# sakarias88/racer-tracer

Hardware: AMD Instinct MI355X
Metric: Msamples/s (W*H*spp/s) at 1920x1080 (higher is better)
Workload: dtype f64; 1 GPU; cornell_box.yml 1920x1080 1024spp max_depth 20; strip_rows=8, parallelism=image rows interleaved over 1 GPU(s)

## Files before the change

### racer-tracer_amd/csrc/rt_api.hip

```cpp
#include <hip/hip_runtime.h>
#include <stdint.h>
#include <stdio.h>
#include <string.h>
#include <algorithm>
#include <cmath>
#include <atomic>
#include <string>
#include <vector>
#include <thread>
#include <chrono>
#include "rt_scene.h"

extern "C" hipError_t rtdev_launch_post_rgba8(const RtToneMap *tm, const double *rgb, size_t n_pixels, uint8_t *rgba,
                                              double *mapped, hipStream_t stream);

using rtapi::Cancel;
using rtapi::Delivery;
using rtapi::chunk_plan;
using rtapi::fail;
using rtapi::owned_rows_of;

namespace {

int fill_args(const RtScene *s, const RtCamera *c, const RtRenderParams *p, rtdev::TraceArgs &a) {
// ... 184 lines not shown
    a.slice_rows = a.owned_rows;
    const size_t slice_elems = (size_t)p->width * (size_t)a.slice_rows * 3;
    if (b.partial.count < slice_elems * (size_t)a.total_chunks) RT_HIP(b.partial.alloc(slice_elems * (size_t)a.total_chunks));
    if (b.queue.count < n_launches) RT_HIP(b.queue.alloc(n_launches));
    a.partial = b.partial.ptr;
    RT_HIP(hipMemsetAsync(b.segments.ptr, 0, rtdev::RT_STAT_SLOTS * sizeof(unsigned long long), stream));
#ifdef RT_PROFILE_REGIONS
    RT_HIP(hipMemsetAsync(b.segments.ptr + rtdev::RT_STAT_WALL + 0, 0xff, sizeof(unsigned long long), stream));
    RT_HIP(hipMemsetAsync(b.segments.ptr + rtdev::RT_STAT_WALL + 2, 0xff, sizeof(unsigned long long), stream));
#endif
    RT_HIP(hipMemsetAsync(b.queue.ptr, 0, sizeof(unsigned int) * b.queue.count, stream));
    const int rc = order_bvh_for_camera(s, camera, stream);
    if (rc != RT_OK) return rc;
    RT_HIP(hipEventRecord(b.ev_begin, stream));
    return RT_OK;
}

int launch_pool(RtScene *s, rtdev::TraceArgs &a, const std::vector<int> &starts, int first_chunk, int n_chunks, int index,
                unsigned max_blocks, hipStream_t stream, const uint32_t *tile_list = nullptr, uint32_t n_list = 0) {
    if (tile_list && (a.n_regions > 1 || n_list > (uint32_t)a.n_tiles))
        return fail(RT_ERR_INVALID_ARGUMENT, "a tile list is for one-region launches, at most one entry per tile");
    a.sample_begin = starts[(size_t)first_chunk];
    a.sample_end = starts[(size_t)(first_chunk + n_chunks)];
    a.n_chunks = n_chunks;
    a.chunk_base = first_chunk;
    a.tile_list = tile_list;
    a.n_list = tile_list ? n_list : 0u;
    const uint32_t tiles = tile_list ? n_list : (uint32_t)a.n_tiles;
    a.n_items = (uint32_t)a.n_chunks * tiles;
    if ((uint64_t)a.n_chunks * (uint64_t)tiles >= 0x40000000ull)
        return fail(RT_ERR_UNSUPPORTED, "more than 2^30 work items in one launch");
    a.queue = s->buf.queue.ptr + index;
    const unsigned blocks = std::min(max_blocks, (a.n_items + 3) / 4);
    RT_HIP(s->kernels->trace_pool(&a, s->prims_class, s->textured, s->specular, s->use_bvh, blocks, stream));
    return RT_OK;
}

int enqueue_pool(RtScene *s, rtdev::TraceArgs &a, const RtCamera *camera, const RtRenderParams *p, double *out_device,
                 hipStream_t stream, int batch, const Cancel &cancel, const Delivery *delivery, int out_col_step,
                 int out_cols, int &launches) {
    std::vector<int> starts;
    unsigned max_blocks = 0;
    int rc = setup_pool_grid(s, a, p, starts, max_blocks);
    if (rc != RT_OK) return rc;
    const int total_chunks = a.total_chunks;
    const std::vector<rtapi::Launch> plan = rtapi::plan_launches(starts, batch);
    if (delivery) {
        if (plan.size() != 1 || p->scale > 1) return fail(RT_ERR_UNSUPPORTED, "a delivering launch is one whole-frame launch");
        if ((rc = setup_delivery(s, a, *delivery, total_chunks, stream)) != RT_OK) return rc;
    }
    rtapi::RenderBuffers &b = s->buf;
    if ((rc = pool_prologue(s, a, camera, p, plan.size(), cancel.armed() || (delivery && delivery->cancellable), stream)) != RT_OK)
        return rc;
    int chunks_done = 0;
    for (const rtapi::Launch &l : plan) {
        if (cancel.raised()) return RT_ERR_CANCEL_EVENT;
        if ((rc = launch_pool(s, a, starts, l.first_chunk, l.n_chunks, launches, max_blocks, stream)) != RT_OK) return rc;
        chunks_done += a.n_chunks;
        ++launches;
    }
    RT_HIP(hipEventRecord(b.ev_traced, stream));
    if (!delivery)
        RT_HIP(s->kernels->resolve_chunks(b.partial.ptr, out_device, p->width, p->height, chunks_done, a.slice_rows, a.strip_rows,
                                          a.strip_count, a.strip_index, a.step_x, a.step_y, a.cover_w, a.cover_h, out_col_step,
                                          out_cols, p->samples, stream));
    RT_HIP(hipEventRecord(b.ev_resolved, stream));
    return RT_OK;
// ... 261 lines not shown
```

### racer-tracer_amd/csrc/rt_pool_coop.h

```cpp
#pragma once
#include "rt_pool_lds.h"

namespace RT_KNS {

__device__ __forceinline__ int lane_rank(uint64_t mask) {
    return (int)__builtin_amdgcn_mbcnt_hi((uint32_t)(mask >> 32), __builtin_amdgcn_mbcnt_lo((uint32_t)mask, 0u));
}

__device__ __forceinline__ void post_request(SphereSlot *slot, const ScatterPrefix &P, uint32_t base) {
    __hip_atomic_store(&slot->b, P.b, __ATOMIC_RELAXED, __HIP_MEMORY_SCOPE_WAVEFRONT);
    __hip_atomic_store(&slot->y, P.y, __ATOMIC_RELAXED, __HIP_MEMORY_SCOPE_WAVEFRONT);
    __hip_atomic_store(&slot->x, P.x, __ATOMIC_RELAXED, __HIP_MEMORY_SCOPE_WAVEFRONT);
    __hip_atomic_store(&slot->w, P.w, __ATOMIC_RELAXED, __HIP_MEMORY_SCOPE_WAVEFRONT);
    __hip_atomic_store(&slot->z, P.z, __ATOMIC_RELAXED, __HIP_MEMORY_SCOPE_WAVEFRONT);
    __hip_atomic_store(&slot->base, base, __ATOMIC_RELAXED, __HIP_MEMORY_SCOPE_WAVEFRONT);
}
__device__ __forceinline__ void move_masked(const d3 &p, uint64_t mask, d3 &v) {
    uint64_t saved;
    asm volatile("s_and_saveexec_b64 %[saved], %[mask]\n\t"
                 "v_mov_b64 %[x], %[px]\n\t"
                 "v_mov_b64 %[y], %[py]\n\t"
                 "v_mov_b64 %[z], %[pz]\n\t"
                 "s_mov_b64 exec, %[saved]"
                 : [x] "+v"(v.x), [y] "+v"(v.y), [z] "+v"(v.z), [saved] "=&s"(saved)
                 : [mask] "s"(mask), [px] "v"(p.x), [py] "v"(p.y), [pz] "v"(p.z)
                 : "scc");
}
__device__ __forceinline__ void increment_masked(uint32_t &v, uint64_t mask) {
    asm("v_addc_co_u32 %[v], vcc, 0, %[v], %[mask]" : [v] "+v"(v) : [mask] "s"(mask) : "vcc");
}
__device__ __forceinline__ uint64_t lowest_in_groups(uint64_t x, int lg) {
    const int q = 1 << lg;
    uint64_t low = 1;
#pragma unroll
    for (int k = 0; k < 6; ++k) low |= low << ((q << k) & 63);
    const uint64_t top = low << (q - 1);
    return x & (((~x & ~top) + low) ^ (~x & top));
}

template <bool PAIRS>
__device__ __forceinline__ void closest_hit_rects(const Prim *table, const d3 &o, const d3 &d, const d3 &inv_d, double &best_t, int &best) {
    auto test_plane = [&](auto axis, const Prim &P, int i) {
#ifndef RT_EXACT_DIV
        rect_closest_update<decltype(axis)::value>(P.p[0], P.p[1], P.p[2], P.p[3], P.p[4], o, d, inv_d, 0.001, best_t, best, i);
        return;
#endif
        double t;
        if (rect_t<true>(decltype(axis)::value, P.p[0], P.p[1], P.p[2], P.p[3], P.p[4], o, d, inv_d, 0.001, best_t, t)) {
            best_t = t;
            best = i;
        }
    };
    const Prim *rec = table;
    int i = 0;
    auto group = [&](auto axis, int end) {
        if (PAIRS) {
            for (; i + 1 < end; i += 2, rec += 2) {
                const Prim pa = load_prim_uniform(rec, 0), pb = load_prim_uniform(rec, 1);
                test_plane(axis, pa, i);
                test_plane(axis, pb, i + 1);
            }
            if (i < end) {
                test_plane(axis, load_prim_uniform(rec, 0), i);
                ++i;
                ++rec;
            }
        } else {
            for (; i < end; ++i, ++rec) test_plane(axis, load_prim_uniform(rec, 0), i);
        }
    };
    const RT_CONSTANT TraceArgs *KB = kernargs_here();
    const int end_xy = KB->rect_end[0], end_xz = KB->rect_end[1], end_yz = KB->rect_end[2];
    group(std::integral_constant<int, 2>(), end_xy);
    group(std::integral_constant<int, 1>(), end_xz);
    group(std::integral_constant<int, 0>(), end_yz);
}

template <int MAX_ROUNDS>
__device__ __forceinline__ uint64_t coop_random_in_unit_sphere(uint64_t pending, uint32_t pixel, uint32_t sample, uint32_t seg,
                                                           uint32_t &base, uint32_t k0, uint32_t k1, int lane,
                                                           SphereSlot *slot, d3 &result) {
    uint64_t have = 0;
    const ScatterPrefix own = scatter_prefix(pixel, sample, seg, k0, k1);
    for (int round = 0; round < MAX_ROUNDS && pending != 0; ++round) {
        const int n = __popcll(pending);
        if (round > 0 && n < 8) break;
        const int lg = n > 32 ? 0 : (n > 16 ? 1 : (n > 8 ? 2 : (n > 4 ? 3 : (n > 2 ? 4 : (n > 1 ? 5 : 6)))));
        d3 cand;
        uint64_t take;
        if (lg == 0) {
            const d3 p = sphere_candidate(philox_from_prefix(own, base, k0, k1));
            cand = p;
            take = pending;
            const uint64_t inside = ballot(len2(p) < 1.0);
            have |= pending & inside;
            pending &= ~inside;
            if (__builtin_amdgcn_inverse_ballot_w64(pending)) base += 1u;
        } else {
            const bool need = __builtin_amdgcn_inverse_ballot_w64(pending);
            const int rank = lane_rank(pending);
            if (need) post_request(slot + rank, own, base);
// ... 127 lines not shown
```

### racer-tracer_amd/csrc/rt_pool_lds.h

```cpp
#pragma once
#include "rt_trace_common.h"

namespace RT_KNS {

struct NoiseSlots {
    double p[8][3];
    int depth[8];
    int perlin[8];
    double term[8][8];
};
struct alignas(16) Req4 {
    uint32_t x, y, z, w;
};
struct alignas(8) SphereSlot {
    uint32_t b, y, x, w, z, base;
};
static_assert(sizeof(SphereSlot) == 3 * sizeof(double), "a slot holds the request or the sample");

template <bool TEXTURED> union SamplerScratch {
    Req4 req[32];
    SphereSlot sphere[32];
    NoiseSlots noise;
};
template <> union SamplerScratch<false> {
    Req4 req[32];
    SphereSlot sphere[32];
};

struct alignas(16) ItemInfo {
    int chunk, tx, ty, tile_py0, region, reg_tiles, rows_aligned, _pad;
};

template <bool TEXTURED, int NBUF, bool OVERLAP> struct WaveLds {
    double base[OVERLAP ? 1 : 64][3];
    double u[OVERLAP ? 64 : 1];
    double sum[OVERLAP ? 128 : 64][3];
    SamplerScratch<TEXTURED> scratch;
    uint8_t pix_of[64];
    double v[NBUF][64];
    ItemInfo info[2];
    double ulc[3];
};

enum : uint32_t { RING_SLOTS = 92u };
struct PretraceLds {
    double cam_origin[3], bg_top[3];
    double u[64];
    double sum[64][3];
    SamplerScratch<false> scratch;
    uint8_t pix_of[64];
    double ring_v[RING_SLOTS];
    double ring_t[RING_SLOTS];
    uint32_t ring_w[RING_SLOTS];
    uint16_t ring_best[RING_SLOTS];
    uint32_t n_started;
    ItemInfo info[1];
    double ulc[3];
};

}
```

### racer-tracer_amd/csrc/rt_primary_bounds.h

```cpp
#pragma once
#include <cmath>
#include <stdint.h>

namespace rtdev {

struct PixelRect {
    int32_t px0, px1, py0, py1;
};

inline PixelRect primary_bounds(const double origin[3], const double ulc[3], const double horizontal[3], const double vertical[3],
                                double lens_radius, int width, int height, const double mn[3], const double mx[3]) {
    const PixelRect whole = {0, width - 1, 0, height - 1};
    const double kPad = 1.0;
    if (width < 2 || height < 2) return whole;
    if (!(lens_radius == 0.0)) return whole;
    for (int k = 0; k < 3; ++k) {
        if (!std::isfinite(origin[k]) || !std::isfinite(ulc[k]) || !std::isfinite(horizontal[k]) || !std::isfinite(vertical[k]))
            return whole;
        if (!std::isfinite(mn[k]) || !std::isfinite(mx[k]) || mn[k] > mx[k]) return whole;
    }
    const double a[3] = {horizontal[0], horizontal[1], horizontal[2]};
    const double b[3] = {-vertical[0], -vertical[1], -vertical[2]};
    const double r[3] = {origin[0] - ulc[0], origin[1] - ulc[1], origin[2] - ulc[2]};
    auto det3 = [](const double p[3], const double q[3], const double s[3]) {
        return p[0] * (q[1] * s[2] - q[2] * s[1]) - p[1] * (q[0] * s[2] - q[2] * s[0]) + p[2] * (q[0] * s[1] - q[1] * s[0]);
    };
    auto norm3 = [](const double p[3]) { return std::sqrt(p[0] * p[0] + p[1] * p[1] + p[2] * p[2]); };
    double u_min = INFINITY, u_max = -INFINITY, v_min = INFINITY, v_max = -INFINITY;
    for (int corner = 0; corner < 8; ++corner) {
        double c[3];
        for (int k = 0; k < 3; ++k) c[k] = -(((corner >> k) & 1 ? mx[k] : mn[k]) - origin[k]);
        const double det = det3(a, b, c);
        if (!std::isfinite(det) || !(std::fabs(det) > 1e-9 * norm3(a) * norm3(b) * norm3(c))) return whole;
        const double u = det3(r, b, c) / det, v = det3(a, r, c) / det, lambda = det3(a, b, r) / det;
        if (!std::isfinite(u) || !std::isfinite(v) || !std::isfinite(lambda) || !(lambda > 0.0)) return whole;
        u_min = std::fmin(u_min, u);
        u_max = std::fmax(u_max, u);
        v_min = std::fmin(v_min, v);
        v_max = std::fmax(v_max, v);
    }
    auto low = [&](double t, int n) { return (int32_t)std::fmin(std::fmax(std::floor(t * (double)(n - 1)) - 1.0 - kPad, 0.0), (double)n); };
    auto high = [&](double t, int n) { return (int32_t)std::fmax(std::fmin(std::ceil(t * (double)(n - 1)) + kPad, (double)(n - 1)), -1.0); };
    return PixelRect{low(u_min, width), high(u_max, width), low(v_min, height), high(v_max, height)};
}

}
```

### racer-tracer_amd/csrc/rt_scene.h

```cpp
#pragma once
#include <hip/hip_runtime.h>
#include <stdint.h>
#include <string>
#include <vector>
#include "rt_device_types.h"
#include "rt_bvh.h"
#include "rt_error.h"
#include "rt_plan.h"
#include "../../include/rt_abi.h"

#define RT_LAUNCHER_LIST(X)                                                                                                \
    X(trace, rtdev_launch_trace, hipError_t,                                                                               \
      (const rtdev::TraceArgs *args, int prims_class, int textured, int specular, hipStream_t stream))                     \
    X(resolve, rtdev_launch_resolve, hipError_t,                                                                           \
      (const double *accum, double *out, int width, int height, int strip_rows, int strip_count, int strip_index,         \
       int samples, hipStream_t stream))                                                                                   \
    X(pool_blocks_per_cu, rtdev_pool_blocks_per_cu, int,                                                                   \
      (int prims_class, int textured, int specular, int bvh, size_t dyn_lds))                                              \
    X(pool_static_lds, rtdev_pool_static_lds, int, (int prims_class, int textured, int specular, int bvh))                 \
    X(trace_pool, rtdev_launch_trace_pool, hipError_t,                                                                     \
      (const rtdev::TraceArgs *args, int prims_class, int textured, int specular, int bvh, unsigned blocks,               \
       hipStream_t stream))                                                                                                \
    X(resolve_chunks, rtdev_launch_resolve_chunks, hipError_t,                                                             \
      (const double *partial, double *out, int width, int height, int n_chunks, int slice_rows, int strip_rows,           \
       int strip_count, int strip_index, int step_x, int step_y, int cover_w, int cover_h, int out_col_step, int out_cols, \
       int samples, hipStream_t stream))                                                                                   \
    X(fold_chunks, rtdev_launch_fold_chunks, hipError_t,                                                                   \
      (const double *partial, double *running, double *out, size_t n, int c0, int c1, int samples_done,                   \
       hipStream_t stream))                                                                                                \
    X(fold_adaptive, rtdev_launch_fold_adaptive, hipError_t, (const rtdev::AdaptiveFold *f, hipStream_t stream))           \
    X(nee, rtdev_launch_nee, hipError_t,                                                                                   \
      (const rtdev::TraceArgs *args, const rtdev::NeeArgs *nee, int prims_class, int textured, int specular, int bvh,     \
       hipStream_t stream))                                                                                                \
    X(nee_pass, rtdev_launch_nee_pass, hipError_t,                                                                         \
      (const rtdev::TraceArgs *args, const rtdev::NeeArgs *nee, int prims_class, int textured, int specular, int bvh,     \
       hipStream_t stream))                                                                                                \
    X(nee_chunk, rtdev_launch_nee_chunk, hipError_t,                                                                       \
      (const double *running, double *boundary, double *squares, size_t n, int samples, hipStream_t stream))              \
    X(nee_decide, rtdev_launch_nee_decide, hipError_t, (const rtdev::NeeDecide *f, hipStream_t stream))                    \
    X(nee_stream, rtdev_launch_nee_stream, hipError_t,                                                                     \
      (const rtdev::TraceArgs *args, const rtdev::NeeArgs *nee, int prims_class, int textured, int specular, int bvh,     \
       unsigned blocks, hipStream_t stream))                                                                               \
    X(nee_stream_blocks_per_cu, rtdev_nee_stream_blocks_per_cu, int,                                                       \
      (int prims_class, int textured, int specular, int bvh))                                                              \
    X(nee_stream_chunk, rtdev_nee_stream_chunk, int, (void))
#define RT_DECLARE_LAUNCHER(member, name, ret, params) \
    extern "C" ret name params;                        \
    extern "C" ret name##_exact params;
RT_LAUNCHER_LIST(RT_DECLARE_LAUNCHER)
#undef RT_DECLARE_LAUNCHER

namespace rtapi {

struct Launchers {
#define RT_LAUNCHER_MEMBER(member, name, ret, params) ret(*member) params;
// ... 101 lines not shown
        for (hipEvent_t *evs : {ev_pass_begin, ev_pass_traced, ev_folded, ev_counted, ev_copied})
            for (int k = 0; k < 3; ++k)
                if (evs[k]) (void)hipEventDestroy(evs[k]);
        if (stream_copy) (void)hipStreamDestroy(stream_copy);
        *this = RenderBuffers();
    }
};

}

extern "C" hipError_t rtdev_launch_guides(const rtdev::TraceArgs *args, const RtGuides *guides, hipStream_t stream);
extern "C" hipError_t rtdev_launch_denoise_step(const RtDenoiseParams *d, int step, int width, int height, const double *in,
                                                const RtGuides *guides, double *out, hipStream_t stream);

struct RtScene {
    int device = 0;
    rtapi::DevBuf<rtdev::Prim> prims;
    rtapi::DevBuf<rtdev::Texture> textures;
    rtapi::DevBuf<rtdev::Image> images;
    rtapi::DevBuf<rtdev::Perlin> perlins;
    std::vector<uint8_t *> image_pixels;
    int n_prims = 0, n_materials = 0, n_textures = 0, n_images = 0, n_perlins = 0;
    int perlin_identity = 1;
    rtdev::Background bg;
    int prims_class = 2;
    int rect_end[3] = {0, 0, 0};
    int sphere_end = 0;
    int box_end = 0;
    int textured = 0;
    double radiance_bound = 0.0;
    int specular = 0;
    int has_moving = 0;
    double box_mn[3] = {1.0, 1.0, 1.0}, box_mx[3] = {-1.0, -1.0, -1.0};

    int use_bvh = 0;
    rtapi::DevBuf<rtdev::BvhNode> bvh_nodes;
    rtapi::DevBuf<rtdev::BvhNode> bvh_nodes_ordered;
    rtapi::DevBuf<int32_t> bvh_prim_index;
    rtapi::DevBuf<rtdev::LeafGeo> leaf_geo;
    double leaf_time_a = 0.0, leaf_inv_dt = 1.0;
    int n_bvh_nodes = 0;
    double bvh_root_mn[3] = {0, 0, 0}, bvh_root_mx[3] = {0, 0, 0}, bvh_center[3] = {0, 0, 0};
    bool bvh_nodes_in_lds = false;
    rtdev::BvhBuild bvh_host;
    double bvh_ordered_for[3] = {0, 0, 0};
    bool bvh_is_ordered = false;
    std::vector<rtdev::BvhNode> bvh_ordered_nodes[2];
    int bvh_upload_slot = 0;

    bool use_v1 = false;
    bool exact = false;
    const rtapi::Launchers *kernels = nullptr;
    bool gather_staged = false;
    int num_cus = 0, pool_blocks_per_cu = 1;
    int pool_blocks_per_cu_lens = 1;
    int pool_static_lds = 0;
    size_t pool_dyn_lds = 0, pool_dyn_lds_lens = 0;

    std::vector<int32_t> lights;
    rtapi::DevBuf<int32_t> nee_slot, nee_prim;

    rtapi::RenderBuffers buf;
    bool has_stats = false;
    int last_launches = 0;
    bool summed_times = false;
    double summed_kernel_ms = 0.0, summed_resolve_ms = 0.0;
// ... 75 lines not shown
```

### racer-tracer_amd/csrc/rt_scene_create.hip

```cpp
#include <hip/hip_runtime.h>
#include <stdint.h>
#include <string.h>
#include <memory>
#include <mutex>
#include <string>
#include <vector>
#include "rt_scene.h"

using rtapi::DevBuf;
using rtapi::fail;

namespace {
struct CachedSet {
    int device;
    rtapi::RenderBuffers buf;
};
std::mutex g_cache_mutex;
std::vector<CachedSet> g_cache;
const size_t kCachedSetsPerDevice = 2;

void render_cache_put(RtScene *s) {
    if (s->buf.complete()) {
        std::lock_guard<std::mutex> lock(g_cache_mutex);
        size_t held = 0;
// ... 159 lines not shown

    std::vector<rtdev::Prim> prims = rtapi::pack_prims(d);
    s->radiance_bound = rtapi::scene_radiance_bound(d);
    const std::vector<rtdev::Perlin> perlins = rtapi::pack_perlins(d, s->perlin_identity);
    const rtapi::Selection sel = rtapi::select_variant(d);
    s->prims_class = sel.prims_class;
    s->textured = sel.textured;
    s->specular = sel.specular;
    s->has_moving = sel.has_moving;
    rtapi::scene_bounds(d, s->box_mn, s->box_mx);
    s->use_bvh = d->n_primitives > rtapi::kBvhThreshold;
    if (opt.closest_hit != RT_HIT_AUTO) s->use_bvh = opt.closest_hit == RT_HIT_BVH && d->n_primitives > 0;
    if (s->radiance_bound == 0.0 && !s->use_v1 && (s->use_bvh || s->prims_class == 2)) s->exact = true;
    s->kernels = s->exact ? &kExactLaunchers : &kFastLaunchers;
    if (!s->use_bvh && (size_t)d->n_primitives * sizeof(rtdev::Prim) > rtapi::kLinearTableBytes)
        return fail(RT_ERR_UNSUPPORTED, "RT_HIT_LINEAR: the primitive table does not fit in LDS");

    std::vector<int32_t> order((size_t)d->n_primitives);
    for (size_t j = 0; j < order.size(); ++j) order[j] = (int32_t)j;
    rtdev::BvhBuild bvh;
    rtapi::LeafTable leaves;
    if (s->use_bvh) {
        bvh = choose_bvh(d, s);
        order.assign(bvh.prim_index.begin(), bvh.prim_index.end());
        std::vector<rtdev::Prim> ordered(prims.size());
        for (size_t j = 0; j < bvh.prim_index.size(); ++j) ordered[j] = prims[(size_t)bvh.prim_index[j]];
        prims.swap(ordered);
        leaves = rtapi::leaf_geometry(prims);
    } else {
        const rtapi::LinearGroups groups = rtapi::group_linear_table(prims, order);
        for (int g = 0; g < 3; ++g) s->rect_end[g] = groups.rect_end[g];
        s->sphere_end = groups.sphere_end;
        s->box_end = groups.box_end;
    }
    const rtapi::LightTables lights = rtapi::light_tables(d, order, rtapi::kMaxLights);

    std::vector<rtdev::Image> images;
    if ((rc = upload_images(d, s, images)) != RT_OK) return rc;
    const std::vector<rtdev::Texture> textures = rtapi::pack_textures(d, images);
    if (s->use_bvh && (rc = upload_bvh(s, bvh, leaves)) != RT_OK) return rc;
    if ((rc = rtapi::build_light_list(s, lights)) != RT_OK) return rc;
    if ((rc = upload(s->prims, prims)) != RT_OK) return rc;
    if ((rc = upload(s->textures, textures)) != RT_OK) return rc;
    if ((rc = upload(s->images, images)) != RT_OK) return rc;
    if ((rc = upload(s->perlins, perlins)) != RT_OK) return rc;
    s->n_prims = d->n_primitives;
    s->n_materials = d->n_materials;
    s->n_textures = d->n_textures;
    s->n_images = d->n_images;
    s->n_perlins = d->n_perlins;
    s->bg.kind = d->background.kind;
    for (int k = 0; k < 3; ++k) {
        s->bg.top[k] = d->background.top[k];
        s->bg.bottom[k] = d->background.bottom[k];
    }
    if ((rc = size_pool(s)) != RT_OK) return rc;
    if ((rc = acquire_render_buffers(s)) != RT_OK) return rc;
    *out = half_built.release();
    return RT_OK;
}

}

extern "C" {

void rt_scene_destroy(RtScene *s) {
// ... 78 lines not shown
```

### racer-tracer_amd/csrc/rt_trace_pool_kernel.hip

```cpp
#include <cstddef>
#include <type_traits>
#include "rt_trace_common.h"
#include "rt_variant_dispatch.h"
#include "rt_pool_profile.h"
#include "rt_pool_lds.h"
#include "rt_pool_coop.h"
#include "rt_pool_deliver.h"

#ifndef RT_OCC_TEX
#define RT_OCC_TEX 4
#endif
#ifndef RT_OCC_TEX_BVH
#define RT_OCC_TEX_BVH 4
#endif
#ifndef RT_OCC_TEX_ANY
#define RT_OCC_TEX_ANY 4
#endif
#ifndef RT_OCC_SPEC
#define RT_OCC_SPEC 5
#endif
#ifndef RT_OCC_ANY
#define RT_OCC_ANY 5
#endif
#ifndef RT_OCC_PLAIN
#define RT_OCC_PLAIN 7
#endif
namespace RT_KNS {

template <int PRIMS, bool TEXTURED, bool SPECULAR, bool BVH>
__global__ __launch_bounds__(256, TEXTURED ? (PRIMS == PRIMS_ANY ? (BVH ? RT_OCC_TEX_BVH : RT_OCC_TEX_ANY) : RT_OCC_TEX) : (BVH ? 4 : (PRIMS == PRIMS_ANY ? RT_OCC_ANY : (SPECULAR ? RT_OCC_SPEC : RT_OCC_PLAIN)))) void k_trace_pool_f64(const TraceArgs A) {
    constexpr int NBUF = BVH ? 1 : 2;
#if defined(RT_EXACT_DIV) || defined(RT_NO_OVERLAP)
    constexpr bool OVERLAP = false;
#else
    constexpr bool OVERLAP = BVH || PRIMS == PRIMS_ANY;
#endif
#ifdef RT_NO_PRETRACE
    constexpr bool PRETRACE = false;
#else
    constexpr bool PRETRACE = PRIMS == PRIMS_RECTS && !TEXTURED && !SPECULAR && !BVH;
#endif
    using Lds = std::conditional_t<PRETRACE, PretraceLds, WaveLds<TEXTURED, NBUF, OVERLAP>>;
    __shared__ Lds lds_all[4];
    extern __shared__ __align__(16) unsigned char dyn_lds[];
    struct PerlinGradients {
        double ranvec[256][3];
    };
    static_assert(offsetof(Perlin, ranvec) == 0, "the gradients lead the Perlin record");
    const Perlin *lds_perlin = nullptr;
    if (TEXTURED) {
        if (A.perlin_in_lds) {
            const size_t at = BVH ? (size_t)A.bvh_lds_nodes * sizeof(BvhNode)
                                  : (size_t)A.n_prims * sizeof(Prim) + (size_t)A.n_textures * sizeof(Texture);
            const uint64_t *src = reinterpret_cast<const uint64_t *>(A.perlins);
            uint64_t *dst = reinterpret_cast<uint64_t *>(dyn_lds + at);
            for (int i = threadIdx.x; i < (int)(sizeof(PerlinGradients) / 8); i += 256) dst[i] = src[i];
            lds_perlin = reinterpret_cast<const Perlin *>(dyn_lds + at);
        }
        __syncthreads();
    }
    double (*lens)[64][2] = nullptr;
    if (A.lens_lds) {
        size_t at = BVH ? (size_t)A.bvh_lds_nodes * sizeof(BvhNode)
// ... 106 lines not shown
        uint32_t tile = local - chunk * reg_tiles;
        if (tile_list != nullptr) tile = (uint32_t)__builtin_amdgcn_readfirstlane((int)tile_list[tile]);
        const int ty = reg_ty0 + (int)(tile / (uint32_t)reg_ntx);
        const int tx = reg_tx0 + (int)(tile % (uint32_t)reg_ntx);
        const int cur = (int)(state >> 6) & 1;
        int n_smp;
        {
            const RT_CONSTANT TraceArgs *K = kernargs_here();
            smp0 = K->chunk_start[A.chunk_base + (int)chunk];
            n_smp = K->chunk_start[A.chunk_base + (int)chunk + 1] - smp0;
        }

        const bool rows_aligned = A.strip_count <= 1 || (A.strip_rows & 7) == 0;
        tile_py0 = ty * 8 * A.step_y;
        if (A.strip_count > 1 && rows_aligned) {
            const int q = (ty * 8) / A.strip_rows;
            tile_py0 = (q * A.strip_count + A.strip_index) * A.strip_rows + (ty * 8 - q * A.strip_rows);
        }
        const int my_px = (tx * 8 + (lane & 7)) * A.step_x;
        const int my_vrow = ty * 8 + (lane >> 3);
        int my_py = tile_py0 + (lane >> 3) * A.step_y;
        if (!rows_aligned)
            my_py = ((my_vrow / A.strip_rows) * A.strip_count + A.strip_index) * A.strip_rows + my_vrow % A.strip_rows;
        const bool my_valid = my_px < A.cover_w && my_vrow < A.owned_rows && my_py < A.height;
        my_pixel = (uint32_t)my_py * (uint32_t)A.width + (uint32_t)my_px;
        const uint64_t valid_mask = ballot(my_valid);
        n_valid = __popcll(valid_mask);
        bool culled = false;
        if constexpr (PRETRACE) {
            const RT_CONSTANT TraceArgs *K = kernargs_here();
            const int x0 = K->cull_px0, x1 = K->cull_px1, y0 = K->cull_py0, y1 = K->cull_py1;
            const uint64_t seen = valid_mask & ballot(my_px >= x0) & ballot(my_px <= x1) & ballot(my_py >= y0) & ballot(my_py <= y1);
            culled = seen == 0ull && K->bg.kind != RT_BG_SKY && K->max_depth >= 1;
        }
        {
            if (!culled) {
                uint32_t pixel_stream = RT_RNG_SAMPLE_PIXEL;
                if constexpr (PRETRACE) asm volatile("" : "+s"(pixel_stream));
                PathRng prng{my_pixel, pixel_stream, A.seed_lo, A.seed_hi};
                u4 bj = prng.block(0, RT_RNG_PIXEL, 0);
                const RT_CONSTANT TraceArgs *K = kernargs_here();
                const double u = div_by((double)my_px + u53(bj.a, bj.b), (double)(A.width - 1), K->inv_width_m1);
                if constexpr (OVERLAP || PRETRACE) {
                    L.u[lane] = u;
                } else {
                    const d3 base = ld3(K->cam.ulc) + u * ld3(K->cam.horizontal);
                    L.base[lane][0] = base.x;
                    L.base[lane][1] = base.y;
                    L.base[lane][2] = base.z;
                }
            }
            unsigned long long zero = FIXED_SUMS ? 0ull - (unsigned long long)n_smp * 0x4330000000000000ull : 0ull;
            if constexpr (PRETRACE) asm volatile("" : "+v"(zero));
            unsigned long long *sum = reinterpret_cast<unsigned long long *>(L.sum[cur * 64 + lane]);
            sum[0] = zero;
            sum[1] = zero;
            sum[2] = zero;
            if (my_valid) L.pix_of[lane_rank(valid_mask)] = lane;
            if (lane == 0) L.info[cur] = ItemInfo{(int)chunk, tx, ty, tile_py0, region, (int)reg_tiles, rows_aligned ? 1 : 0, 0};
        }
        if constexpr (PRETRACE) {
            if (culled) {
                const d3 bg = ld3(L.bg_top);
                if (bg.x != 0.0 || bg.y != 0.0 || bg.z != 0.0)
                    for (int k = 0; k < n_smp; ++k) {
                        atomicAdd(&L.sum[lane_of_wave][0], bg.x);
// ... 118 lines not shown
                atomicAdd(&L.sum[pix_b][0], one);
                atomicAdd(&L.sum[pix_b][1], one);
                atomicAdd(&L.sum[pix_b][2], one);
            }
            if (lane == 0) L.n_started += (uint32_t)__popcll(in_pool);
            next += (uint32_t)__popcll(in_pool);
            return;
        }
        const u4 bc = philox4x32(pixel_b, sample_b, RT_RNG_CAMERA, 0u, A.seed_lo, A.seed_hi);
        const uint32_t in_ring = min(b << 6, total) - next;
        uint32_t park = ring_head + in_ring + (uint32_t)lane;
        if (park >= RING_SLOTS) park -= RING_SLOTS;
        d3 bo, bd;
        {
            const double v = div_by((double)py_b + u53(bc.a, bc.b), (double)(A.height - 1), K->inv_height_m1);
            double lx, ly;
            asm volatile("" : "=v"(lx), "=v"(ly));
            if (kernargs_here()->lens_lds != 0) {
                lx = ly = 0.0;
                uint32_t w_here = w;
                asm volatile("" : "+v"(w_here));
                coop_random_in_unit_disk(w_here < total, pixel_b, sample_b, A.seed_lo, A.seed_hi, lane, L.scratch.req, lx, ly);
                lx = lx * K->cam.lens_radius;
                ly = ly * K->cam.lens_radius;
                lens_ring[park][0] = lx;
                lens_ring[park][1] = ly;
            }
            L.ring_v[park] = v;
            camera_ray(pix_b, v, lx, ly, bo, bd);
        }
        double best_t = __builtin_inf();
        int best = -1;
        increment_masked(n_segments, in_pool);
        closest_hit_rects<false>(A.prims, bo, bd, rcp3(bd), best_t, best);
        d3 C = ld3(L.bg_top);
        if (kernargs_here()->bg.kind == RT_BG_SKY) {
            const double t = 0.5 * (unit_fast(bd).y + 1.0);
            C = (1.0 - t) * C + t * ld3(kernargs_here()->bg.bottom);
        }
        const uint64_t hit = in_pool & ballot(best >= 0);
        int kind;
        asm volatile("" : "=v"(kind));
        if (__builtin_amdgcn_inverse_ballot_w64(hit)) {
            const Material &M = lds_prims[best].mat;
            kind = M.kind;
            C = ld3(M.color);
        }
        asm volatile("" : "+v"(kind));
        const uint64_t light = hit & ballot(kind == RT_MAT_DIFFUSE_LIGHT);
        const uint64_t ends = kernargs_here()->max_depth <= 1 ? in_pool : (in_pool & ~hit) | light;
        const uint64_t lives = in_pool & ~ends;
        if (__builtin_amdgcn_inverse_ballot_w64(ends)) {
            atomicAdd(&L.sum[pix_b][0], C.x);
            atomicAdd(&L.sum[pix_b][1], C.y);
            atomicAdd(&L.sum[pix_b][2], C.z);
        }
        if (lane == 0) L.n_started += (uint32_t)__popcll(in_pool);
        uint32_t slot = ring_head + in_ring + (uint32_t)lane_rank(lives);
        if (slot >= RING_SLOTS) slot -= RING_SLOTS;
        if (__builtin_amdgcn_inverse_ballot_w64(lives)) {
            const double v = L.ring_v[park];
            double lx, ly;
            asm volatile("" : "=v"(lx), "=v"(ly));
            if (kernargs_here()->lens_lds != 0) {
                lx = lens_ring[park][0];
                ly = lens_ring[park][1];
            }
            asm volatile("" ::: "memory");
            L.ring_v[slot] = v;
            L.ring_t[slot] = best_t;
            L.ring_w[slot] = w;
            L.ring_best[slot] = (uint16_t)best;
            if (kernargs_here()->lens_lds != 0) {
                lens_ring[slot][0] = lx;
                lens_ring[slot][1] = ly;
            }
        }
        next += (uint32_t)__popcll(ends);
        }
    };

    uint64_t alive_m = 0;
    int spix = 0;
    PathRng rng{0, 0, A.seed_lo, A.seed_hi};
    d3 o = mk(0, 0, 0), d = o, T = o;
    uint32_t seg = 0;
    double ray_time = 0.0;
    uint64_t waiting_m = 0;
// ... 526 lines not shown
    if (lane == 0 && total_segments) atomicAdd(A.segments + RT_STAT_SEGMENTS, total_segments);
    if constexpr (PRETRACE) {
        int first = lane_of_wave;
        asm volatile("" : "+v"(first));
        n_started = first == 0 ? L.n_started : 0u;
    }
    unsigned long long started = n_started;
#pragma unroll
    for (int off = 32; off > 0; off >>= 1) started += __shfl_down(started, off, 64);
    if (lane == 0 && started) atomicAdd(A.segments + RT_STAT_SAMPLES, started);
}

}

#if defined(RT_BB_COUNT) && !defined(RT_EXACT_DIV)
enum { RT_BB_MAX = 8192 };
extern "C" {
__device__ __attribute__((used)) unsigned long long rt_bb_counts[RT_BB_MAX];
int rtdev_bb_counts(unsigned long long *out, int n, int reset) {
    if (n > RT_BB_MAX) n = RT_BB_MAX;
    if (hipDeviceSynchronize() != hipSuccess) return -1;
    if (out && hipMemcpyFromSymbol(out, HIP_SYMBOL(rt_bb_counts), (size_t)n * sizeof(unsigned long long)) != hipSuccess) return -1;
    if (reset) {
        static unsigned long long zeros[RT_BB_MAX];
        if (hipMemcpyToSymbol(HIP_SYMBOL(rt_bb_counts), zeros, sizeof zeros) != hipSuccess) return -1;
    }
    return n;
}
}
#endif

namespace {
template <int PRIMS, bool TEXTURED, bool SPECULAR, bool BVH> struct PoolVariant {
    static void launch(const rtdev::TraceArgs &a, unsigned blocks, hipStream_t stream) {
        const size_t dyn = rtdev::pool_lds_layout(BVH, TEXTURED, a.n_prims, a.n_textures, a.bvh_lds_nodes, a.perlin_in_lds, a.lens_lds,
                                                  a.time_lds).bytes;
        hipLaunchKernelGGL((RT_KNS::k_trace_pool_f64<PRIMS, TEXTURED, SPECULAR, BVH>), dim3(blocks), dim3(256), dyn, stream, a);
    }
    static int blocks_per_cu(size_t dyn_lds) {
        int n = 0;
        if (hipOccupancyMaxActiveBlocksPerMultiprocessor(&n, RT_KNS::k_trace_pool_f64<PRIMS, TEXTURED, SPECULAR, BVH>, 256, dyn_lds) != hipSuccess)
            return 1;
        hipFuncAttributes attr;
        if (hipFuncGetAttributes(&attr, (const void *)RT_KNS::k_trace_pool_f64<PRIMS, TEXTURED, SPECULAR, BVH>) == hipSuccess) {
            const size_t granules = (attr.sharedSizeBytes + dyn_lds + 1279) / 1280;
            if (granules > 0 && (int)(128 / granules) < n) n = (int)(128 / granules);
        }
        return n < 0 ? 0 : n;
    }
    static int static_lds() {
        hipFuncAttributes attr;
        if (hipFuncGetAttributes(&attr, (const void *)RT_KNS::k_trace_pool_f64<PRIMS, TEXTURED, SPECULAR, BVH>) != hipSuccess) return -1;
        return (int)attr.sharedSizeBytes;
    }
};
}

extern "C" int RT_LAUNCHER(rtdev_pool_blocks_per_cu)(int prims_class, int textured, int specular, int bvh, size_t dyn_lds) {
    return rtdev::dispatch_variant<PoolVariant>(prims_class, textured != 0, specular != 0, bvh != 0,
                                                [dyn_lds](auto v) { return decltype(v)::blocks_per_cu(dyn_lds); });
}

extern "C" int RT_LAUNCHER(rtdev_pool_static_lds)(int prims_class, int textured, int specular, int bvh) {
    return rtdev::dispatch_variant<PoolVariant>(prims_class, textured != 0, specular != 0, bvh != 0,
                                                [](auto v) { return decltype(v)::static_lds(); });
}

extern "C" hipError_t RT_LAUNCHER(rtdev_launch_trace_pool)(const rtdev::TraceArgs *args, int prims_class, int textured, int specular,
                                              int bvh, unsigned blocks, hipStream_t stream) {
    if (blocks == 0 || args->n_items == 0) return hipSuccess;
    rtdev::dispatch_variant<PoolVariant>(prims_class, textured != 0, specular != 0, bvh != 0, [&](auto v) {
        decltype(v)::launch(*args, blocks, stream);
    });
    return hipGetLastError();
}
```

Baseline: 41730 Msamples/s.

## Cull per-rectangle primary ray tests using host-projected screen bounds

The host projects each axis-aligned rectangle's corners onto the image plane and passes per-rect pixel bounds as a second kernel argument. Each wave then builds a bitmask of the rectangles its pixels can possibly see and skips plane tests for the others in the primary-hit loop. This targets the intersection cost of camera rays in an all-rectangle scene like the Cornell box. It adds ballot loops per item and LDS state, and relies on padding and reading kernarg memory past TraceArgs. The LDS atomic address computation is also rewritten with 32-bit offsets.

```diff
diff --git a/racer-tracer_amd/csrc/rt_api.hip b/racer-tracer_amd/csrc/rt_api.hip
--- a/racer-tracer_amd/csrc/rt_api.hip
+++ b/racer-tracer_amd/csrc/rt_api.hip
@@ -240,7 +240,10 @@
         return fail(RT_ERR_UNSUPPORTED, "more than 2^30 work items in one launch");
     a.queue = s->buf.queue.ptr + index;
     const unsigned blocks = std::min(max_blocks, (a.n_items + 3) / 4);
-    RT_HIP(s->kernels->trace_pool(&a, s->prims_class, s->textured, s->specular, s->use_bvh, blocks, stream));
+    const rtdev::PrimaryRects rects = rtdev::primary_rects(a.cam.origin, a.cam.ulc, a.cam.horizontal, a.cam.vertical, a.width, a.height,
+                                                           rtdev::PixelRect{a.cull_px0, a.cull_px1, a.cull_py0, a.cull_py1},
+                                                           s->primary_rect_geo.data(), (int)s->primary_rect_geo.size());
+    RT_HIP(s->kernels->trace_pool(&a, &rects, s->prims_class, s->textured, s->specular, s->use_bvh, blocks, stream));
     return RT_OK;
 }
 
diff --git a/racer-tracer_amd/csrc/rt_pool_coop.h b/racer-tracer_amd/csrc/rt_pool_coop.h
--- a/racer-tracer_amd/csrc/rt_pool_coop.h
+++ b/racer-tracer_amd/csrc/rt_pool_coop.h
@@ -1,5 +1,6 @@
 #pragma once
 #include "rt_pool_lds.h"
+#include "rt_primary_bounds.h"
 
 namespace RT_KNS {
 
@@ -29,6 +30,10 @@
 __device__ __forceinline__ void increment_masked(uint32_t &v, uint64_t mask) {
     asm("v_addc_co_u32 %[v], vcc, 0, %[v], %[mask]" : [v] "+v"(v) : [mask] "s"(mask) : "vcc");
 }
+static_assert(sizeof(TraceArgs) % alignof(rtdev::PrimaryRects) == 0, "no padding between the kernel's two arguments");
+__device__ __forceinline__ const RT_CONSTANT rtdev::PrimaryRects *primary_rects_here() {
+    return (const RT_CONSTANT rtdev::PrimaryRects *)((const RT_CONSTANT unsigned char *)kernargs_here() + sizeof(TraceArgs));
+}
 __device__ __forceinline__ uint64_t lowest_in_groups(uint64_t x, int lg) {
     const int q = 1 << lg;
     uint64_t low = 1;
@@ -38,8 +43,10 @@
     return x & (((~x & ~top) + low) ^ (~x & top));
 }
 
+static_assert(rtdev::RT_PRIMARY_RECTS <= 32, "a rect mask is one 32-bit word");
 template <bool PAIRS>
-__device__ __forceinline__ void closest_hit_rects(const Prim *table, const d3 &o, const d3 &d, const d3 &inv_d, double &best_t, int &best) {
+__device__ __forceinline__ void closest_hit_rects(const Prim *table, const d3 &o, const d3 &d, const d3 &inv_d, double &best_t, int &best,
+                                                  uint32_t rect_mask = ~0u) {
     auto test_plane = [&](auto axis, const Prim &P, int i) {
 #ifndef RT_EXACT_DIV
         rect_closest_update<decltype(axis)::value>(P.p[0], P.p[1], P.p[2], P.p[3], P.p[4], o, d, inv_d, 0.001, best_t, best, i);
@@ -66,7 +73,13 @@
                 ++rec;
             }
         } else {
-            for (; i < end; ++i, ++rec) test_plane(axis, load_prim_uniform(rec, 0), i);
+            const int n = end - i;
+            if (n > 0 && n < 32 && ((rect_mask >> (i & 31)) & ((1u << n) - 1u)) == 0u) {
+                i = end;
+                rec = reinterpret_cast<const Prim *>(reinterpret_cast<const unsigned char *>(rec) + (uint32_t)n * (uint32_t)sizeof(Prim));
+            }
+            for (; i < end; ++i, ++rec)
+                if ((rect_mask >> (i & 31)) & 1u) test_plane(axis, load_prim_uniform(rec, 0), i);
         }
     };
     const RT_CONSTANT TraceArgs *KB = kernargs_here();
diff --git a/racer-tracer_amd/csrc/rt_pool_lds.h b/racer-tracer_amd/csrc/rt_pool_lds.h
--- a/racer-tracer_amd/csrc/rt_pool_lds.h
+++ b/racer-tracer_amd/csrc/rt_pool_lds.h
@@ -54,6 +54,7 @@
     uint32_t ring_w[RING_SLOTS];
     uint16_t ring_best[RING_SLOTS];
     uint32_t n_started;
+    uint32_t rect_mask;
     ItemInfo info[1];
     double ulc[3];
 };
diff --git a/racer-tracer_amd/csrc/rt_primary_bounds.h b/racer-tracer_amd/csrc/rt_primary_bounds.h
--- a/racer-tracer_amd/csrc/rt_primary_bounds.h
+++ b/racer-tracer_amd/csrc/rt_primary_bounds.h
@@ -8,17 +8,9 @@
     int32_t px0, px1, py0, py1;
 };
 
-inline PixelRect primary_bounds(const double origin[3], const double ulc[3], const double horizontal[3], const double vertical[3],
-                                double lens_radius, int width, int height, const double mn[3], const double mx[3]) {
-    const PixelRect whole = {0, width - 1, 0, height - 1};
+inline bool project_points(const double origin[3], const double ulc[3], const double horizontal[3], const double vertical[3],
+                           int width, int height, const double (*points)[3], int n, PixelRect &out) {
     const double kPad = 1.0;
-    if (width < 2 || height < 2) return whole;
-    if (!(lens_radius == 0.0)) return whole;
-    for (int k = 0; k < 3; ++k) {
-        if (!std::isfinite(origin[k]) || !std::isfinite(ulc[k]) || !std::isfinite(horizontal[k]) || !std::isfinite(vertical[k]))
-            return whole;
-        if (!std::isfinite(mn[k]) || !std::isfinite(mx[k]) || mn[k] > mx[k]) return whole;
-    }
     const double a[3] = {horizontal[0], horizontal[1], horizontal[2]};
     const double b[3] = {-vertical[0], -vertical[1], -vertical[2]};
     const double r[3] = {origin[0] - ulc[0], origin[1] - ulc[1], origin[2] - ulc[2]};
@@ -27,21 +19,85 @@
     };
     auto norm3 = [](const double p[3]) { return std::sqrt(p[0] * p[0] + p[1] * p[1] + p[2] * p[2]); };
     double u_min = INFINITY, u_max = -INFINITY, v_min = INFINITY, v_max = -INFINITY;
-    for (int corner = 0; corner < 8; ++corner) {
+    for (int i = 0; i < n; ++i) {
         double c[3];
-        for (int k = 0; k < 3; ++k) c[k] = -(((corner >> k) & 1 ? mx[k] : mn[k]) - origin[k]);
+        for (int k = 0; k < 3; ++k) c[k] = -(points[i][k] - origin[k]);
         const double det = det3(a, b, c);
-        if (!std::isfinite(det) || !(std::fabs(det) > 1e-9 * norm3(a) * norm3(b) * norm3(c))) return whole;
+        if (!std::isfinite(det) || !(std::fabs(det) > 1e-9 * norm3(a) * norm3(b) * norm3(c))) return false;
         const double u = det3(r, b, c) / det, v = det3(a, r, c) / det, lambda = det3(a, b, r) / det;
-        if (!std::isfinite(u) || !std::isfinite(v) || !std::isfinite(lambda) || !(lambda > 0.0)) return whole;
+        if (!std::isfinite(u) || !std::isfinite(v) || !std::isfinite(lambda) || !(lambda > 0.0)) return false;
         u_min = std::fmin(u_min, u);
         u_max = std::fmax(u_max, u);
         v_min = std::fmin(v_min, v);
         v_max = std::fmax(v_max, v);
     }
-    auto low = [&](double t, int n) { return (int32_t)std::fmin(std::fmax(std::floor(t * (double)(n - 1)) - 1.0 - kPad, 0.0), (double)n); };
-    auto high = [&](double t, int n) { return (int32_t)std::fmax(std::fmin(std::ceil(t * (double)(n - 1)) + kPad, (double)(n - 1)), -1.0); };
-    return PixelRect{low(u_min, width), high(u_max, width), low(v_min, height), high(v_max, height)};
+    auto low = [&](double t, int m) { return (int32_t)std::fmin(std::fmax(std::floor(t * (double)(m - 1)) - 1.0 - kPad, 0.0), (double)m); };
+    auto high = [&](double t, int m) { return (int32_t)std::fmax(std::fmin(std::ceil(t * (double)(m - 1)) + kPad, (double)(m - 1)), -1.0); };
+    out = PixelRect{low(u_min, width), high(u_max, width), low(v_min, height), high(v_max, height)};
+    return true;
+}
+
+inline PixelRect primary_bounds(const double origin[3], const double ulc[3], const double horizontal[3], const double vertical[3],
+                                double lens_radius, int width, int height, const double mn[3], const double mx[3]) {
+    const PixelRect whole = {0, width - 1, 0, height - 1};
+    if (width < 2 || height < 2) return whole;
+    if (!(lens_radius == 0.0)) return whole;
+    for (int k = 0; k < 3; ++k) {
+        if (!std::isfinite(origin[k]) || !std::isfinite(ulc[k]) || !std::isfinite(horizontal[k]) || !std::isfinite(vertical[k]))
+            return whole;
+        if (!std::isfinite(mn[k]) || !std::isfinite(mx[k]) || mn[k] > mx[k]) return whole;
+    }
+    double corners[8][3];
+    for (int corner = 0; corner < 8; ++corner)
+        for (int k = 0; k < 3; ++k) corners[corner][k] = (corner >> k) & 1 ? mx[k] : mn[k];
+    PixelRect rect;
+    return project_points(origin, ulc, horizontal, vertical, width, height, corners, 8, rect) ? rect : whole;
+}
+
+struct RectGeo {
+    int32_t axis;
+    double a0, a1, b0, b1, k;
+};
+
+enum { RT_PRIMARY_RECTS = 16 };
+
+struct alignas(8) PrimaryRects {
+    int32_t n, _pad;
+    PixelRect r[RT_PRIMARY_RECTS];
+};
+
+inline bool is_whole_frame(const PixelRect &r, int width, int height) {
+    return r.px0 == 0 && r.px1 == width - 1 && r.py0 == 0 && r.py1 == height - 1;
+}
+
+inline PixelRect primary_rect_bounds(const double origin[3], const double ulc[3], const double horizontal[3], const double vertical[3],
+                                     int width, int height, const PixelRect &scene, const RectGeo &g) {
+    const PixelRect whole = {0, width - 1, 0, height - 1};
+    if (width < 2 || height < 2 || is_whole_frame(scene, width, height)) return whole;
+    if (g.axis < 0 || g.axis > 2) return whole;
+    if (!std::isfinite(g.a0) || !std::isfinite(g.a1) || !std::isfinite(g.b0) || !std::isfinite(g.b1) || !std::isfinite(g.k)) return whole;
+    if (g.a0 > g.a1 || g.b0 > g.b1) return whole;
+    const int ia = g.axis == 0 ? 1 : 0, ib = g.axis == 2 ? 1 : 2;
+    double corners[4][3];
+    for (int corner = 0; corner < 4; ++corner) {
+        corners[corner][g.axis] = g.k;
+        corners[corner][ia] = corner & 1 ? g.a1 : g.a0;
+        corners[corner][ib] = corner & 2 ? g.b1 : g.b0;
+    }
+    PixelRect rect;
+    return project_points(origin, ulc, horizontal, vertical, width, height, corners, 4, rect) ? rect : whole;
+}
+
+inline PrimaryRects primary_rects(const double origin[3], const double ulc[3], const double horizontal[3], const double vertical[3],
+                                  int width, int height, const PixelRect &scene, const RectGeo *rects, int n_rects) {
+    PrimaryRects out;
+    out._pad = 0;
+    const bool off = n_rects <= 0 || n_rects > RT_PRIMARY_RECTS || width < 2 || height < 2 || is_whole_frame(scene, width, height);
+    out.n = off ? 0 : n_rects;
+    for (int i = 0; i < RT_PRIMARY_RECTS; ++i)
+        out.r[i] = !off && i < n_rects ? primary_rect_bounds(origin, ulc, horizontal, vertical, width, height, scene, rects[i])
+                                       : PixelRect{0, width - 1, 0, height - 1};
+    return out;
 }
 
 }
diff --git a/racer-tracer_amd/csrc/rt_scene.h b/racer-tracer_amd/csrc/rt_scene.h
--- a/racer-tracer_amd/csrc/rt_scene.h
+++ b/racer-tracer_amd/csrc/rt_scene.h
@@ -19,8 +19,8 @@
       (int prims_class, int textured, int specular, int bvh, size_t dyn_lds))                                              \
     X(pool_static_lds, rtdev_pool_static_lds, int, (int prims_class, int textured, int specular, int bvh))                 \
     X(trace_pool, rtdev_launch_trace_pool, hipError_t,                                                                     \
-      (const rtdev::TraceArgs *args, int prims_class, int textured, int specular, int bvh, unsigned blocks,               \
-       hipStream_t stream))                                                                                                \
+      (const rtdev::TraceArgs *args, const rtdev::PrimaryRects *rects, int prims_class, int textured, int specular,       \
+       int bvh, unsigned blocks, hipStream_t stream))                                                                      \
     X(resolve_chunks, rtdev_launch_resolve_chunks, hipError_t,                                                             \
       (const double *partial, double *out, int width, int height, int n_chunks, int slice_rows, int strip_rows,           \
        int strip_count, int strip_index, int step_x, int step_y, int cover_w, int cover_h, int out_col_step, int out_cols, \
@@ -188,6 +188,7 @@
     int specular = 0;
     int has_moving = 0;
     double box_mn[3] = {1.0, 1.0, 1.0}, box_mx[3] = {-1.0, -1.0, -1.0};
+    std::vector<rtdev::RectGeo> primary_rect_geo;
 
     int use_bvh = 0;
     rtapi::DevBuf<rtdev::BvhNode> bvh_nodes;
diff --git a/racer-tracer_amd/csrc/rt_scene_create.hip b/racer-tracer_amd/csrc/rt_scene_create.hip
--- a/racer-tracer_amd/csrc/rt_scene_create.hip
+++ b/racer-tracer_amd/csrc/rt_scene_create.hip
@@ -215,6 +215,12 @@
         for (int g = 0; g < 3; ++g) s->rect_end[g] = groups.rect_end[g];
         s->sphere_end = groups.sphere_end;
         s->box_end = groups.box_end;
+        const int n_rects = groups.rect_end[2];
+        if (n_rects == d->n_primitives && n_rects <= rtdev::RT_PRIMARY_RECTS)
+            for (int j = 0; j < n_rects; ++j) {
+                const rtdev::Prim &q = prims[(size_t)j];
+                s->primary_rect_geo.push_back(rtdev::RectGeo{j < groups.rect_end[0] ? 2 : (j < groups.rect_end[1] ? 1 : 0), q.p[0], q.p[1], q.p[2], q.p[3], q.p[4]});
+            }
     }
     const rtapi::LightTables lights = rtapi::light_tables(d, order, rtapi::kMaxLights);
 
diff --git a/racer-tracer_amd/csrc/rt_trace_pool_kernel.hip b/racer-tracer_amd/csrc/rt_trace_pool_kernel.hip
--- a/racer-tracer_amd/csrc/rt_trace_pool_kernel.hip
+++ b/racer-tracer_amd/csrc/rt_trace_pool_kernel.hip
@@ -1,6 +1,7 @@
 #include <cstddef>
 #include <type_traits>
 #include "rt_trace_common.h"
+#include "rt_primary_bounds.h"
 #include "rt_variant_dispatch.h"
 #include "rt_pool_profile.h"
 #include "rt_pool_lds.h"
@@ -28,7 +29,7 @@
 namespace RT_KNS {
 
 template <int PRIMS, bool TEXTURED, bool SPECULAR, bool BVH>
-__global__ __launch_bounds__(256, TEXTURED ? (PRIMS == PRIMS_ANY ? (BVH ? RT_OCC_TEX_BVH : RT_OCC_TEX_ANY) : RT_OCC_TEX) : (BVH ? 4 : (PRIMS == PRIMS_ANY ? RT_OCC_ANY : (SPECULAR ? RT_OCC_SPEC : RT_OCC_PLAIN)))) void k_trace_pool_f64(const TraceArgs A) {
+__global__ __launch_bounds__(256, TEXTURED ? (PRIMS == PRIMS_ANY ? (BVH ? RT_OCC_TEX_BVH : RT_OCC_TEX_ANY) : RT_OCC_TEX) : (BVH ? 4 : (PRIMS == PRIMS_ANY ? RT_OCC_ANY : (SPECULAR ? RT_OCC_SPEC : RT_OCC_PLAIN)))) void k_trace_pool_f64(const TraceArgs A, const rtdev::PrimaryRects) {
     constexpr int NBUF = BVH ? 1 : 2;
 #if defined(RT_EXACT_DIV) || defined(RT_NO_OVERLAP)
     constexpr bool OVERLAP = false;
@@ -201,6 +202,17 @@
             const int x0 = K->cull_px0, x1 = K->cull_px1, y0 = K->cull_py0, y1 = K->cull_py1;
             const uint64_t seen = valid_mask & ballot(my_px >= x0) & ballot(my_px <= x1) & ballot(my_py >= y0) & ballot(my_py <= y1);
             culled = seen == 0ull && K->bg.kind != RT_BG_SKY && K->max_depth >= 1;
+            uint32_t rect_mask = ~0u;
+            if (!culled) {
+                const RT_CONSTANT rtdev::PrimaryRects *R = primary_rects_here();
+                const int n_rects = R->n;
+                for (int i = 0; i < n_rects; ++i) {
+                    const int rx0 = R->r[i].px0, rx1 = R->r[i].px1, ry0 = R->r[i].py0, ry1 = R->r[i].py1;
+                    const uint64_t sees = valid_mask & ballot(my_px >= rx0) & ballot(my_px <= rx1) & ballot(my_py >= ry0) & ballot(my_py <= ry1);
+                    if (sees == 0ull) rect_mask &= ~(1u << i);
+                }
+            }
+            if (lane == 0) L.rect_mask = rect_mask;
         }
         {
             if (!culled) {
@@ -385,7 +397,8 @@
         double best_t = __builtin_inf();
         int best = -1;
         increment_masked(n_segments, in_pool);
-        closest_hit_rects<false>(A.prims, bo, bd, rcp3(bd), best_t, best);
+        const uint32_t rect_mask = (uint32_t)__builtin_amdgcn_readfirstlane((int)L.rect_mask);
+        closest_hit_rects<false>(A.prims, bo, bd, rcp3(bd), best_t, best, rect_mask);
         d3 C = ld3(L.bg_top);
         if (kernargs_here()->bg.kind == RT_BG_SKY) {
             const double t = 0.5 * (unit_fast(bd).y + 1.0);
@@ -404,9 +417,10 @@
         const uint64_t ends = kernargs_here()->max_depth <= 1 ? in_pool : (in_pool & ~hit) | light;
         const uint64_t lives = in_pool & ~ends;
         if (__builtin_amdgcn_inverse_ballot_w64(ends)) {
-            atomicAdd(&L.sum[pix_b][0], C.x);
-            atomicAdd(&L.sum[pix_b][1], C.y);
-            atomicAdd(&L.sum[pix_b][2], C.z);
+            double *const sum = reinterpret_cast<double *>(reinterpret_cast<unsigned char *>(&L.sum[0][0]) + (uint32_t)pix_b * (uint32_t)sizeof(L.sum[0]));
+            atomicAdd(sum + 0, C.x);
+            atomicAdd(sum + 1, C.y);
+            atomicAdd(sum + 2, C.z);
         }
         if (lane == 0) L.n_started += (uint32_t)__popcll(in_pool);
         uint32_t slot = ring_head + in_ring + (uint32_t)lane_rank(lives);
@@ -999,10 +1013,10 @@
 
 namespace {
 template <int PRIMS, bool TEXTURED, bool SPECULAR, bool BVH> struct PoolVariant {
-    static void launch(const rtdev::TraceArgs &a, unsigned blocks, hipStream_t stream) {
+    static void launch(const rtdev::TraceArgs &a, const rtdev::PrimaryRects &r, unsigned blocks, hipStream_t stream) {
         const size_t dyn = rtdev::pool_lds_layout(BVH, TEXTURED, a.n_prims, a.n_textures, a.bvh_lds_nodes, a.perlin_in_lds, a.lens_lds,
                                                   a.time_lds).bytes;
-        hipLaunchKernelGGL((RT_KNS::k_trace_pool_f64<PRIMS, TEXTURED, SPECULAR, BVH>), dim3(blocks), dim3(256), dyn, stream, a);
+        hipLaunchKernelGGL((RT_KNS::k_trace_pool_f64<PRIMS, TEXTURED, SPECULAR, BVH>), dim3(blocks), dim3(256), dyn, stream, a, r);
     }
     static int blocks_per_cu(size_t dyn_lds) {
         int n = 0;
@@ -1033,11 +1047,11 @@
                                                 [](auto v) { return decltype(v)::static_lds(); });
 }
 
-extern "C" hipError_t RT_LAUNCHER(rtdev_launch_trace_pool)(const rtdev::TraceArgs *args, int prims_class, int textured, int specular,
-                                              int bvh, unsigned blocks, hipStream_t stream) {
+extern "C" hipError_t RT_LAUNCHER(rtdev_launch_trace_pool)(const rtdev::TraceArgs *args, const rtdev::PrimaryRects *rects, int prims_class,
+                                              int textured, int specular, int bvh, unsigned blocks, hipStream_t stream) {
     if (blocks == 0 || args->n_items == 0) return hipSuccess;
     rtdev::dispatch_variant<PoolVariant>(prims_class, textured != 0, specular != 0, bvh != 0, [&](auto v) {
-        decltype(v)::launch(*args, blocks, stream);
+        decltype(v)::launch(*args, *rects, blocks, stream);
     });
     return hipGetLastError();
 }
```

Result: faster. 42750 Msamples/s, median of 6 (+2.4%).
